# mengcaopku/DCNet

Measured on AMD Instinct MI355X. Metric: clips/sec (T=8, 416x416, bs8) fwd+bwd, higher is better.
Workload: dtype f32; 1 GPU; T=8 416x416 bs8/GPU L=20 fp32, 64 img/GPU/step as pairs, fwd+5 losses+bwd+RMSprop; arith=f16x2-split MFMA, fp32 accumulate, parallelism=dp1, ranks_seen=1, reducer=none, step=hipGraph replay (fwd+losses+bwd+RMSprop), sampler=mt

## Files before the change

### dcnet_amd/csrc/coattn.hip

```cpp
#include "igemm.h"
#include "prof.h"
#include "coattn.h"

int tn_gemm_batched(const float* A, int lda, long long a_bs, const float* B, int ldb, long long b_bs,
                    float* C, int ldc, long long c_bs, const float* row_scale,
                    int M, int m_ld, int N, int K, int batch, int accumulate, hipStream_t stream,
                    const unsigned* amax_a = nullptr, const unsigned* amax_b = nullptr);

namespace {

constexpr int EXP_ROWS = 32;

typedef _Float16 f16x4c_t __attribute__((ext_vector_type(4)));
constexpr float E_SPLIT_SCALE = 8192.f;
template <bool SPLIT>
__global__ __launch_bounds__(256) void exp_sums_kernel(float* __restrict__ E, int hw, int ldE, float t,
                                                       float* __restrict__ rsum, float* __restrict__ colpart) {
  __shared__ float red[4][EXP_ROWS];
  const int b = blockIdx.y, rb = blockIdx.x;
  const int i0 = rb * EXP_ROWS;
  float* e = E + ((size_t)b * hw + i0) * ldE;
  float racc[EXP_ROWS];
#pragma unroll
  for (int r = 0; r < EXP_ROWS; ++r) racc[r] = 0.f;
  const int nrow = min(EXP_ROWS, hw - i0);
  for (int j = threadIdx.x * 4; j < ldE; j += 1024) {
    f32x4 v[EXP_ROWS];
#pragma unroll
    for (int r = 0; r < EXP_ROWS; ++r)
      v[r] = r < nrow ? *reinterpret_cast<const f32x4*>(e + (size_t)r * ldE + j) : f32x4{0.f, 0.f, 0.f, 0.f};
    f32x4 cs = {0.f, 0.f, 0.f, 0.f};
#pragma unroll
    for (int r = 0; r < EXP_ROWS; ++r) {
      if (r < nrow) {
        f32x4 o;
#pragma unroll
        for (int k = 0; k < 4; ++k) o[k] = (j + k < hw) ? expf(t * v[r][k] - t) : 0.f;
        if constexpr (SPLIT) {
          const f32x4 ts = o * E_SPLIT_SCALE;
          const f16x4c_t h = {(_Float16)ts[0], (_Float16)ts[1], (_Float16)ts[2], (_Float16)ts[3]};
          const f16x4c_t l = {(_Float16)(ts[0] - (float)h[0]), (_Float16)(ts[1] - (float)h[1]), (_Float16)(ts[2] - (float)h[2]),
                              (_Float16)(ts[3] - (float)h[3])};
          unsigned char* run = reinterpret_cast<unsigned char*>(e + (size_t)r * ldE + (j & ~7)) + (j & 4) * 2;
          *reinterpret_cast<f16x4c_t*>(run) = h;
          *reinterpret_cast<f16x4c_t*>(run + 16) = l;
        } else {
          *reinterpret_cast<f32x4*>(e + (size_t)r * ldE + j) = o;
        }
        cs += o; racc[r] += (o[0] + o[1]) + (o[2] + o[3]);
      }
    }
    *reinterpret_cast<f32x4*>(colpart + ((size_t)rb * gridDim.y + b) * ldE + j) = cs;
  }
  const int lane = threadIdx.x & 63, wave = threadIdx.x >> 6;
#pragma unroll
  for (int r = 0; r < EXP_ROWS; ++r) {
    const float s = wave_sum(racc[r]);
    if (lane == 0) red[wave][r] = s;
  }
  __syncthreads();
  if (threadIdx.x < EXP_ROWS && i0 + threadIdx.x < hw)
    rsum[(size_t)b * hw + i0 + threadIdx.x] = 1.f / (red[0][threadIdx.x] + red[1][threadIdx.x] + red[2][threadIdx.x] + red[3][threadIdx.x]);
}

__global__ __launch_bounds__(256) void colsum_inv_kernel(const float* __restrict__ colpart, int nrb, int b, int hw, int ldE,
                                                         float* __restrict__ cinv) {
  const int j = blockIdx.x * 256 + threadIdx.x, bb = blockIdx.y;
  if (j >= hw) return;
  float s = 0.f;
  for (int rb = 0; rb < nrb; ++rb) s += colpart[((size_t)rb * b + bb) * ldE + j];
  cinv[(size_t)bb * hw + j] = 1.f / s;
}

enum { AM_ONE = 0, AM_DO1, AM_DO2, AM_DO1S, AM_DO2S, AM_DA, AM_DP1, AM_DP2, AM_SLOTS };
__global__ __launch_bounds__(256) void amax_init_kernel(unsigned* __restrict__ w) {
  for (int i = threadIdx.x; i < AM_SLOTS * DCN_AMAX_WORDS; i += 256) w[i] = i < DCN_AMAX_WORDS ? 0x3F800000u : 0u;
}

__global__ __launch_bounds__(256) void rowdot_scale_kernel(const float* __restrict__ d, int ldd, int64_t bsd,
                                                           const float* __restrict__ o, int ldo, int64_t bso, int hw,
                                                           const float* __restrict__ inv, int64_t rows, int c,
                                                           float* __restrict__ delta, float* __restrict__ ds,
                                                           unsigned* __restrict__ amax_d, unsigned* __restrict__ amax_ds) {
  __shared__ float red[4];
  const int lane = threadIdx.x & 63;
  const int64_t row = (int64_t)blockIdx.x * 4 + (threadIdx.x >> 6);
  float vmax = 0.f, s = 0.f;
  if (row < rows) {
    const int64_t bb = row / hw, i = row - bb * hw;
    s = inv[row];
    float acc = 0.f;
    for (int k = lane * 4; k < c; k += 256) {
      const f32x4 dv = *reinterpret_cast<const f32x4*>(d + bb * bsd + i * ldd + k);
      const f32x4 ov = *reinterpret_cast<const f32x4*>(o + bb * bso + i * ldo + k);
      acc += dv[0] * ov[0] + dv[1] * ov[1] + dv[2] * ov[2] + dv[3] * ov[3];
      *reinterpret_cast<f32x4*>(ds + row * c + k) = dv * s;
      vmax = fmaxf(fmaxf(vmax, fmaxf(fabsf(dv[0]), fabsf(dv[1]))), fmaxf(fabsf(dv[2]), fabsf(dv[3])));
    }
    acc = wave_sum(acc);
    if (lane == 0) delta[row] = acc;
  }
  const float vs = wave_max(vmax * s);
  amax_update_block(amax_d, vmax, red);
  __syncthreads();
  amax_update_block(amax_ds, vs, red);
}

template <bool ESPLIT, bool OSPLIT = false>
__global__ __launch_bounds__(256) void dA_kernel(const float* __restrict__ E, float* __restrict__ dP1, const float* __restrict__ dP2,
                                                 const float* __restrict__ rinv, const float* __restrict__ cinv,
                                                 const float* __restrict__ d1, const float* __restrict__ d2,
                                                 int hw, int ldE, float t, int64_t total4, unsigned* __restrict__ amax_da) {
  __shared__ float red[4];
  float vmax = 0.f;
  const int l4 = ldE >> 2;
  float s_out = 1.f;
  if constexpr (OSPLIT) {
    const int be = (int)((amax_read(amax_da) >> 23) & 0xFF);
    int ex = (be == 0 || be == 255) ? 0 : 14 - (be - 126);
    ex = ex > 100 ? 100 : (ex < -100 ? -100 : ex);
    s_out = __uint_as_float((unsigned)(ex + 127) << 23);
  }
  for (int64_t idx = (int64_t)blockIdx.x * 256 + threadIdx.x; idx < total4; idx += (int64_t)gridDim.x * 256) {
    const int64_t row = idx / l4;
    const int j = (int)(idx - row * l4) * 4;
    const int64_t bb = row / hw;
    f32x4 e;
    if constexpr (ESPLIT) {
      const unsigned char* run = reinterpret_cast<const unsigned char*>(E + row * ldE + (j & ~7)) + (j & 4) * 2;
      const f16x4c_t h = *reinterpret_cast<const f16x4c_t*>(run), l = *reinterpret_cast<const f16x4c_t*>(run + 16);
#pragma unroll
      for (int k = 0; k < 4; ++k) e[k] = ((float)h[k] + (float)l[k]) * (1.f / E_SPLIT_SCALE);
    } else {
      e = *reinterpret_cast<const f32x4*>(E + row * ldE + j);
    }
    const f32x4 p1 = *reinterpret_cast<const f32x4*>(dP1 + row * ldE + j);
    const f32x4 p2 = *reinterpret_cast<const f32x4*>(dP2 + row * ldE + j);
    const float ri = rinv[row], di = d1[row];
    f32x4 o;
#pragma unroll
    for (int k = 0; k < 4; ++k) {
      float v = 0.f;
      if (j + k < hw) v = t * e[k] * ((p1[k] - di) * ri + (p2[k] - d2[bb * hw + j + k]) * cinv[bb * hw + j + k]);
      o[k] = v;
    }
    if constexpr (OSPLIT) {
      const f32x4 ts = o * s_out;
      const f16x4c_t h = {(_Float16)ts[0], (_Float16)ts[1], (_Float16)ts[2], (_Float16)ts[3]};
      const f16x4c_t l = {(_Float16)(ts[0] - (float)h[0]), (_Float16)(ts[1] - (float)h[1]), (_Float16)(ts[2] - (float)h[2]),
                          (_Float16)(ts[3] - (float)h[3])};
      unsigned char* run = reinterpret_cast<unsigned char*>(dP1 + row * ldE + (j & ~7)) + (j & 4) * 2;
      *reinterpret_cast<f16x4c_t*>(run) = h;
      *reinterpret_cast<f16x4c_t*>(run + 16) = l;
    } else {
      *reinterpret_cast<f32x4*>(dP1 + row * ldE + j) = o;
      vmax = fmaxf(fmaxf(vmax, fmaxf(fabsf(o[0]), fabsf(o[1]))), fmaxf(fabsf(o[2]), fabsf(o[3])));
    }
  }
  if constexpr (!OSPLIT) amax_update_block(amax_da, vmax, red);
}

__global__ __launch_bounds__(64) void da_bound_kernel(const unsigned* __restrict__ a1, const unsigned* __restrict__ a2, float t,
                                                      unsigned* __restrict__ out) {
  const float b = 2.f * t * (__uint_as_float(amax_read(a1)) + __uint_as_float(amax_read(a2)));
  out[threadIdx.x & (DCN_AMAX_WORDS - 1)] = __float_as_uint(b);
}

inline int ld_pad(int hw) { return (hw + 31) / 32 * 32; }

void gemm_params(IgemmParams& p, const float* A, int lda, long long a_bs, const float* B, int ldb, long long b_bs,
                 float* C, int ldc, long long c_bs, int M, int N, int K, int batch) {
  p = IgemmParams{};
  p.osy = p.osx = p.isy = p.isx = 1; p.dense_out = 1;
  p.in = A; p.ldi = lda; p.in_bs = a_bs; p.wt = B; p.ldw = ldb; p.wt_bs = b_bs; p.out = C; p.ldo = ldc; p.out_bs = c_bs;
  p.ldr = ldc;
  p.N = 1; p.Hi = 1; p.Wi = M; p.Ho = 1; p.Wo = M; p.Hs = 1; p.Ws = M; p.M = M;
  p.Ci = K; p.Co = N; p.ntaps = 1; p.batch = batch;
}

}

static bool on_gemm3(int b, int hw, int c) { return c % 32 == 0 && gemm3_applicable(hw, c, hw, b) && gemm3_applicable(hw, hw, c, b); }

int coattn_ld_pad(int hw) { return ld_pad(hw); }
bool coattn_on_gemm3(int b, int hw, int c) { return on_gemm3(b, hw, c); }
unsigned* coattn_ws_amax(float* ws, int b, int hw) { return reinterpret_cast<unsigned*>(ws + (int64_t)cdiv(hw, EXP_ROWS) * b * ld_pad(hw)); }
int coattn_amax_init(unsigned* am, hipStream_t stream) {
  hipLaunchKernelGGL(amax_init_kernel, dim3(1), dim3(256), 0, stream, am);
  DCN_CHECK_LAUNCH("coattn amax_init");
  return DCN_OK;
}
int coattn_exp_sums(float* E, int b, int hw, float temperature, float* rinv, float* cinv, float* ws, bool split, hipStream_t stream) {
  const int ldE = ld_pad(hw), nrb = cdiv(hw, EXP_ROWS);
  const int pid = prof_begin(12, (double)b * hw * ldE * 8.0, stream);
  if (split) hipLaunchKernelGGL(exp_sums_kernel<true>, dim3(nrb, b), dim3(256), 0, stream, E, hw, ldE, temperature, rinv, ws);
  else hipLaunchKernelGGL(exp_sums_kernel<false>, dim3(nrb, b), dim3(256), 0, stream, E, hw, ldE, temperature, rinv, ws);
  prof_end(pid, stream);
  DCN_CHECK_LAUNCH("exp_sums");
  hipLaunchKernelGGL(colsum_inv_kernel, dim3(cdiv(hw, 256), b), dim3(256), 0, stream, ws, nrb, b, hw, ldE, cinv);
  DCN_CHECK_LAUNCH("colsum_inv");
  return DCN_OK;
}

extern "C" int64_t dcn_coattn_fwd_ws(int b, int hw, int c) {
  (void)c;
  return (int64_t)cdiv(hw, EXP_ROWS) * b * ld_pad(hw) + AM_SLOTS * DCN_AMAX_WORDS;
}
extern "C" int64_t dcn_coattn_e_size(int b, int hw) { return (int64_t)b * hw * ld_pad(hw); }
extern "C" int64_t dcn_coattn_saved_size(int b, int hw, int c) {
  return dcn_coattn_e_size(b, hw) + (on_gemm3(b, hw, c) ? (int64_t)2 * b * hw * c : 0);
}

extern "C" int dcn_coattn_fwd(const float* f1, const float* f2, int ldf, int64_t bsf, float* f1_attn, float* f2_attn, int ldo,
                              int64_t bso, float* E, float* rinv, float* cinv, float* ws,
                              int b, int hw, int c, float temperature, void* stream_) {
  hipStream_t stream = (hipStream_t)stream_;
  DCN_CHECK_ARG(f1 && f2 && f1_attn && E && rinv && cinv && ws, "coattn_fwd: null pointer");
  DCN_CHECK_ARG(b > 0 && hw > 0 && c > 0 && c % 32 == 0, "coattn_fwd: bad shape (c=%d must be a multiple of 32)", c);
  if (ldf <= 0) ldf = c;
  if (ldo <= 0) ldo = c;
  DCN_CHECK_ARG(ldf % 4 == 0 && ldo % 4 == 0, "coattn_fwd: ldf/ldo must be multiples of 4");
  if (bsf <= 0) bsf = (int64_t)hw * ldf;
  if (bso <= 0) bso = (int64_t)hw * ldo;
  DCN_CHECK_ARG(bsf % 4 == 0 && bso % 4 == 0, "coattn_fwd: batch strides must be multiples of 4");
  const int ldE = ld_pad(hw);
  unsigned* am = reinterpret_cast<unsigned*>(ws + (int64_t)cdiv(hw, EXP_ROWS) * b * ldE);
  hipLaunchKernelGGL(amax_init_kernel, dim3(1), dim3(256), 0, stream, am);
  DCN_CHECK_LAUNCH("coattn amax_init");
  const unsigned* one = am + AM_ONE * DCN_AMAX_WORDS;
  const int nrb = cdiv(hw, EXP_ROWS);
  const long long bsE = (long long)hw * ldE;
  if (on_gemm3(b, hw, c)) {
    float* f1s = E + dcn_coattn_e_size(b, hw);
    float* f2s = f1s + (int64_t)b * hw * c;
    const long long bss = (long long)hw * c;
    int rc = gemm3_presplit(f1, ldf, bsf, f1s, c, bss, b, hw, c, one, stream);
    if (rc) return rc;
    if ((rc = gemm3_presplit(f2, ldf, bsf, f2s, c, bss, b, hw, c, one, stream))) return rc;
    if ((rc = gemm3_launch(f1s, c, bss, 0, f2s, c, bss, 0, E, ldE, bsE, nullptr, 0, hw, hw, c, b, 0, one, one, stream))) return rc;
    const int pid = prof_begin(12, (double)b * hw * ldE * 8.0, stream);
    hipLaunchKernelGGL(exp_sums_kernel<true>, dim3(nrb, b), dim3(256), 0, stream, E, hw, ldE, temperature, rinv, ws);
    prof_end(pid, stream);
    DCN_CHECK_LAUNCH("exp_sums");
    hipLaunchKernelGGL(colsum_inv_kernel, dim3(cdiv(hw, 256), b), dim3(256), 0, stream, ws, nrb, b, hw, ldE, cinv);
    DCN_CHECK_LAUNCH("colsum_inv");
    if ((rc = gemm3_launch(E, ldE, bsE, 0, f2s, c, bss, 1, f1_attn, ldo, bso, rinv, hw, hw, c, hw, b, 0, one, one, stream))) return rc;
    if (f2_attn) rc = gemm3_launch(E, ldE, bsE, 1, f1s, c, bss, 1, f2_attn, ldo, bso, cinv, hw, hw, c, hw, b, 0, one, one, stream);
    return rc;
  }
  IgemmParams p;
  gemm_params(p, f1, ldf, bsf, f2, ldf, bsf, E, ldE, (long long)hw * ldE, hw, hw, c, b);
  p.amax_a = one; p.amax_b = one;
  int rc = igemm_launch(p, stream);
  if (rc) return rc;
  const int pid = prof_begin(12, (double)b * hw * ldE * 8.0, stream);
  hipLaunchKernelGGL(exp_sums_kernel<false>, dim3(nrb, b), dim3(256), 0, stream, E, hw, ldE, temperature, rinv, ws);
  prof_end(pid, stream);
  DCN_CHECK_LAUNCH("exp_sums");
  hipLaunchKernelGGL(colsum_inv_kernel, dim3(cdiv(hw, 256), b), dim3(256), 0, stream, ws, nrb, b, hw, ldE, cinv);
  DCN_CHECK_LAUNCH("colsum_inv");
  gemm_params(p, E, ldE, (long long)hw * ldE, f2, ldf, bsf, f1_attn, ldo, bso, hw, c, ldE, b);
  p.bmode = 1; p.kvalid = hw; p.row_scale = rinv; p.amax_a = one; p.amax_b = one;
  rc = igemm_launch(p, stream);
  if (rc) return rc;
  if (f2_attn)
    rc = tn_gemm_batched(E, ldE, (long long)hw * ldE, f1, ldf, bsf, f2_attn, ldo, bso,
                         cinv, hw, ldE, c, hw, b, 0, stream, one, one);
  return rc;
}

extern "C" int64_t dcn_coattn_bwd_ws(int b, int hw, int c) {
  return (int64_t)2 * b * hw * ld_pad(hw) + (int64_t)2 * b * hw * c + (int64_t)2 * b * hw + AM_SLOTS * DCN_AMAX_WORDS +
         (on_gemm3(b, hw, c) ? (int64_t)2 * b * hw * c + 4 : 0);
}

extern "C" int dcn_coattn_bwd(const float* f1, const float* f2, int ldf, int64_t bsf,
                              const float* d_f1_attn, const float* d_f2_attn, int lddo, int64_t bsdo,
                              const float* f1_attn, const float* f2_attn, int ldo, int64_t bso,
                              const float* E, const float* rinv, const float* cinv,
                              float* d_f1, float* d_f2, int lddf, int64_t bsdf, int accumulate, float* ws,
                              int b, int hw, int c, float temperature, void* stream_) {
  hipStream_t stream = (hipStream_t)stream_;
  DCN_CHECK_ARG(f1 && f2 && d_f1_attn && d_f2_attn && f1_attn && f2_attn && E && rinv && cinv && d_f1 && d_f2 && ws,
                "coattn_bwd: null pointer");
  DCN_CHECK_ARG(b > 0 && hw > 0 && c > 0 && c % 32 == 0, "coattn_bwd: bad shape");
  if (ldf <= 0) ldf = c;
  if (ldo <= 0) ldo = c;
  if (lddo <= 0) lddo = c;
  if (lddf <= 0) lddf = c;
  if (bsf <= 0) bsf = (int64_t)hw * ldf;
  if (bso <= 0) bso = (int64_t)hw * ldo;
  if (bsdo <= 0) bsdo = (int64_t)hw * lddo;
  if (bsdf <= 0) bsdf = (int64_t)hw * lddf;
  const int ldE = ld_pad(hw);
  const long long rows = (long long)b * hw;
  float* dP1 = ws;
  float* dP2 = dP1 + rows * ldE;
  float* dO1s = dP2 + rows * ldE;
  float* dO2s = dO1s + rows * c;
  float* del1 = dO2s + rows * c;
  float* del2 = del1 + rows;
  unsigned* am = reinterpret_cast<unsigned*>(del2 + rows);
  hipLaunchKernelGGL(amax_init_kernel, dim3(1), dim3(256), 0, stream, am);
  DCN_CHECK_LAUNCH("coattn amax_init");
  auto slot = [&](int i) { return am + i * DCN_AMAX_WORDS; };
  hipLaunchKernelGGL(rowdot_scale_kernel, dim3(cdiv(rows, 4)), dim3(256), 0, stream, d_f1_attn, lddo, bsdo, f1_attn, ldo, bso, hw, rinv, rows, c, del1, dO1s,
                     slot(AM_DO1), slot(AM_DO1S));
  DCN_CHECK_LAUNCH("rowdot_scale");
  hipLaunchKernelGGL(rowdot_scale_kernel, dim3(cdiv(rows, 4)), dim3(256), 0, stream, d_f2_attn, lddo, bsdo, f2_attn, ldo, bso, hw, cinv, rows, c, del2, dO2s,
                     slot(AM_DO2), slot(AM_DO2S));
  DCN_CHECK_LAUNCH("rowdot_scale");
  const int64_t total4 = rows * (ldE / 4);
  int64_t g = (total4 + 255) / 256; if (g > 8192) g = 8192;
  if (g > 1024) g = 1024;
  const long long bsE = (long long)hw * ldE;
  if (on_gemm3(b, hw, c)) {
    float* dO1p = reinterpret_cast<float*>(((uintptr_t)(am + AM_SLOTS * DCN_AMAX_WORDS) + 15) & ~(uintptr_t)15);
    float* dO2p = dO1p + rows * c;
    const float* f1s = E + dcn_coattn_e_size(b, hw);
    const float* f2s = f1s + rows * c;
    const long long bss = (long long)hw * c;
    int rc;
    if ((rc = gemm3_presplit(d_f1_attn, lddo, bsdo, dO1p, c, bss, b, hw, c, slot(AM_DO1), stream))) return rc;
    if ((rc = gemm3_presplit(d_f2_attn, lddo, bsdo, dO2p, c, bss, b, hw, c, slot(AM_DO2), stream))) return rc;
    if ((rc = gemm3_presplit(dO1s, c, bss, dO1s, c, bss, b, hw, c, slot(AM_DO1S), stream))) return rc;
    if ((rc = gemm3_presplit(dO2s, c, bss, dO2s, c, bss, b, hw, c, slot(AM_DO2S), stream))) return rc;
    if ((rc = gemm3_launch(dO1p, c, bss, 0, f2s, c, bss, 0, dP1, ldE, bsE, nullptr, 0, hw, hw, c, b, 0, slot(AM_DO1), slot(AM_ONE), stream, slot(AM_DP1)))) return rc;
    if ((rc = gemm3_launch(f1s, c, bss, 0, dO2p, c, bss, 0, dP2, ldE, bsE, nullptr, 0, hw, hw, c, b, 0, slot(AM_ONE), slot(AM_DO2), stream, slot(AM_DP2)))) return rc;
    hipLaunchKernelGGL(da_bound_kernel, dim3(1), dim3(64), 0, stream, slot(AM_DP1), slot(AM_DP2), temperature, slot(AM_DA));
    DCN_CHECK_LAUNCH("dA bound");
    const int pid_da = prof_begin(31, (double)total4 * 16.0 * 4.0, stream);
    hipLaunchKernelGGL((dA_kernel<true, true>), dim3((int)g), dim3(256), 0, stream, E, dP1, dP2, rinv, cinv, del1, del2, hw, ldE, temperature, total4, slot(AM_DA));
    prof_end(pid_da, stream);
    DCN_CHECK_LAUNCH("dA");
    if ((rc = gemm3_launch(dP1, ldE, bsE, 0, f2s, c, bss, 1, d_f1, lddf, bsdf, nullptr, 0, hw, c, hw, b, accumulate, slot(AM_DA), slot(AM_ONE), stream))) return rc;
    if ((rc = gemm3_launch(E, ldE, bsE, 0, dO2s, c, bss, 1, d_f1, lddf, bsdf, nullptr, 0, hw, c, hw, b, 1, slot(AM_ONE), slot(AM_DO2S), stream))) return rc;
    if ((rc = gemm3_launch(dP1, ldE, bsE, 1, f1s, c, bss, 1, d_f2, lddf, bsdf, nullptr, 0, hw, c, hw, b, accumulate, slot(AM_DA), slot(AM_ONE), stream))) return rc;
    return gemm3_launch(E, ldE, bsE, 1, dO1s, c, bss, 1, d_f2, lddf, bsdf, nullptr, 0, hw, c, hw, b, 1, slot(AM_ONE), slot(AM_DO1S), stream);
  }
  IgemmParams p;
  int rc;
  gemm_params(p, d_f1_attn, lddo, bsdo, f2, ldf, bsf, dP1, ldE, (long long)hw * ldE, hw, hw, c, b);
  p.amax_a = slot(AM_DO1); p.amax_b = slot(AM_ONE);
  if ((rc = igemm_launch(p, stream))) return rc;
  gemm_params(p, f1, ldf, bsf, d_f2_attn, lddo, bsdo, dP2, ldE, (long long)hw * ldE, hw, hw, c, b);
  p.amax_a = slot(AM_ONE); p.amax_b = slot(AM_DO2);
  if ((rc = igemm_launch(p, stream))) return rc;
  const int pid_da = prof_begin(31, (double)total4 * 16.0 * 4.0, stream);
  hipLaunchKernelGGL(dA_kernel<false>, dim3((int)g), dim3(256), 0, stream, E, dP1, dP2, rinv, cinv, del1, del2, hw, ldE, temperature, total4, slot(AM_DA));
  prof_end(pid_da, stream);
  DCN_CHECK_LAUNCH("dA");
  gemm_params(p, dP1, ldE, (long long)hw * ldE, f2, ldf, bsf, d_f1, lddf, bsdf, hw, c, ldE, b);
  p.bmode = 1; p.kvalid = hw; p.accumulate = accumulate; p.amax_a = slot(AM_DA); p.amax_b = slot(AM_ONE);
  if ((rc = igemm_launch(p, stream))) return rc;
  gemm_params(p, E, ldE, (long long)hw * ldE, dO2s, c, (long long)hw * c, d_f1, lddf, bsdf, hw, c, ldE, b);
  p.bmode = 1; p.kvalid = hw; p.accumulate = 1; p.amax_a = slot(AM_ONE); p.amax_b = slot(AM_DO2S);
  if ((rc = igemm_launch(p, stream))) return rc;
  rc = tn_gemm_batched(dP1, ldE, (long long)hw * ldE, f1, ldf, bsf, d_f2, lddf, bsdf,
                       nullptr, hw, ldE, c, hw, b, accumulate, stream, slot(AM_DA), slot(AM_ONE));
  if (rc) return rc;
  return tn_gemm_batched(E, ldE, (long long)hw * ldE, dO1s, c, (long long)hw * c, d_f2, lddf, bsdf,
                         nullptr, hw, ldE, c, hw, b, 1, stream, slot(AM_ONE), slot(AM_DO1S));
}
```

### dcnet_amd/csrc/gemm3.hip

```cpp
#include "igemm.h"
#include "prof.h"

namespace {

typedef _Float16 f16x8_t __attribute__((ext_vector_type(8)));
typedef short s16x4 __attribute__((ext_vector_type(4)));
typedef short s16x8 __attribute__((ext_vector_type(8)));
typedef __attribute__((address_space(3))) void lds_void;

#ifndef G3_ABL
#define G3_ABL 0
#endif
constexpr unsigned G3_OOB = 0x80000000u;
constexpr int G3_BM = 256, G3_BN = 256, G3_STAGES = 4;
constexpr int G3_TILE = 256 * 64;
constexpr int G3_STAGE = 2 * G3_TILE;
constexpr int G3_LDS = G3_STAGES * G3_STAGE;

__device__ __forceinline__ float g3_pow2_scale(unsigned amax_bits) {
  const int be = (int)((amax_bits >> 23) & 0xFF);
  if (be == 0 || be == 255) return 1.f;
  int e = 14 - (be - 126);
  e = e > 100 ? 100 : (e < -100 ? -100 : e);
  return __uint_as_float((unsigned)(e + 127) << 23);
}

struct G3Params {
  const float* A; const float* B; float* C;
  long long a_bs, b_bs, c_bs;
  int lda, ldb, ldc;
  int M, N, K;
  int a_rows, b_rows;
  int a_cols, b_cols;
  int tiles_m, tiles_n;
  const float* row_scale; long long rs_bs;
  int accumulate;
  const unsigned* amax_a; const unsigned* amax_b;
  unsigned* amax_out;
  int var;
  int abl;
};

__device__ __forceinline__ int g3_tswz(int krow) { return (krow & 1) | ((krow & 2) << 1); }

template <bool AT, bool BT, bool H1 = false>
__global__ __launch_bounds__(512, 1) void gemm3_kernel(const G3Params p) {
  extern __shared__ __attribute__((aligned(1024))) unsigned char smem3g[];
  const int tid = threadIdx.x, lane = tid & 63;
  const int wave = __builtin_amdgcn_readfirstlane(tid >> 6);
  const int wm = wave >> 2, wn = wave & 3;
  const int per_batch = p.tiles_m * p.tiles_n;
  const int lin = xcd_remap(blockIdx.x, gridDim.x);
  const int batch = __builtin_amdgcn_readfirstlane(lin / per_batch), t_ = lin - batch * per_batch;
  const int bm = __builtin_amdgcn_readfirstlane(t_ / p.tiles_n), bn = t_ - bm * p.tiles_n;
  const int m0 = bm * G3_BM, n0 = bn * G3_BN;
  const int kslices = (p.K + 15) >> 4;

  const float* a_base = p.A + batch * p.a_bs + (AT ? 0 : (long long)m0 * p.lda);
  const float* b_base = p.B + batch * p.b_bs + (BT ? 0 : (long long)n0 * p.ldb);
  const int a_rows_left = AT ? p.a_rows : p.a_rows - m0, b_rows_left = BT ? p.b_rows : p.b_rows - n0;
  const long long a_bytes = ((long long)(a_rows_left - 1) * p.lda + p.a_cols) * 4, b_bytes = ((long long)(b_rows_left - 1) * p.ldb + p.b_cols) * 4;
  const __amdgpu_buffer_rsrc_t a_rs = __builtin_amdgcn_make_buffer_rsrc((void*)a_base, 0, a_bytes > 0x7FFFFFF0LL ? 0x7FFFFFF0 : (int)a_bytes, 0x00020000);
  const __amdgpu_buffer_rsrc_t b_rs = __builtin_amdgcn_make_buffer_rsrc((void*)b_base, 0, b_bytes > 0x7FFFFFF0LL ? 0x7FFFFFF0 : (int)b_bytes, 0x00020000);

  unsigned voff[4];
  int sstep_a, sstep_b;
#pragma unroll
  for (int e = 0; e < 2; ++e) {
    const int j = 2 * wave + e;
    if (AT) {
      voff[e] = (unsigned)((long long)j * p.lda * 4 + m0 * 4 + ((lane ^ g3_tswz(j)) << 4));
      if (m0 + ((lane ^ g3_tswz(j)) << 2) >= p.a_cols) voff[e] = G3_OOB;
    } else {
      const int row = 16 * j + (lane >> 2), c = (lane & 3) ^ ((row >> 2) & 3);
      voff[e] = row < a_rows_left ? (unsigned)((long long)row * p.lda * 4 + c * 16) : G3_OOB;
    }
    if (BT) {
      voff[2 + e] = (unsigned)((long long)j * p.ldb * 4 + n0 * 4 + ((lane ^ g3_tswz(j)) << 4));
      if (n0 + ((lane ^ g3_tswz(j)) << 2) >= p.b_cols) voff[2 + e] = G3_OOB;
    } else {
      const int row = 16 * j + (lane >> 2), c = (lane & 3) ^ ((row >> 2) & 3);
      voff[2 + e] = row < b_rows_left ? (unsigned)((long long)row * p.ldb * 4 + c * 16) : G3_OOB;
    }
  }
  sstep_a = AT ? 16 * p.lda * 4 : 64;
  sstep_b = BT ? 16 * p.ldb * 4 : 64;
  const int my_dst = 2 * wave * 1024;

  int k_done = 0;
  auto issue_a = [&]() {
    const bool live = k_done < kslices && !(G3_ABL && (p.abl & 1));
    unsigned char* st = smem3g + (k_done & (G3_STAGES - 1)) * G3_STAGE + my_dst;
    int sa_ = live ? k_done * sstep_a : 0;
    if (G3_ABL && (p.abl & 8)) sa_ = 0;
#pragma unroll
    for (int e = 0; e < 2; ++e)
      __builtin_amdgcn_raw_ptr_buffer_load_lds(a_rs, (lds_void*)(st + e * 1024), 16, (int)(live ? voff[e] : G3_OOB), sa_, 0, 0);
  };
  auto issue_b = [&]() {
    const bool live = k_done < kslices && !(G3_ABL && (p.abl & 1));
    unsigned char* st = smem3g + (k_done & (G3_STAGES - 1)) * G3_STAGE + my_dst;
    int sb_ = live ? k_done * sstep_b : 0;
    if (G3_ABL && (p.abl & 8)) sb_ = 0;
#pragma unroll
    for (int e = 0; e < 2; ++e)
      __builtin_amdgcn_raw_ptr_buffer_load_lds(b_rs, (lds_void*)(st + G3_TILE + e * 1024), 16, (int)(live ? voff[2 + e] : G3_OOB), sb_, 0, 0);
    ++k_done;
  };
  auto issue = [&]() { issue_a(); issue_b(); };

  const int g = lane >> 5;
  const int hh = lane >> 5, gg = (lane >> 4) & 1, qq = (lane & 15) >> 2, pp = lane & 3;
  int a_rd[4][2], b_rd[2][2];
#pragma unroll
  for (int mi = 0; mi < 4; ++mi) {
    if (AT) {
      const int c = wm * 128 + mi * 32 + 16 * gg + 4 * pp;
#pragma unroll
      for (int r2 = 0; r2 < 2; ++r2) {
        const int kr = 8 * hh + 4 * r2 + qq;
        a_rd[mi][r2] = kr * 1024 + ((((c >> 3) * 2) ^ g3_tswz(kr)) << 4) + (c & 7) * 2;
      }
    } else {
      const int ar = wm * 128 + mi * 32 + (lane & 31);
      a_rd[mi][0] = ar * 64 + (((2 * g) ^ ((ar >> 2) & 3)) << 4);
      a_rd[mi][1] = ar * 64 + (((2 * g + 1) ^ ((ar >> 2) & 3)) << 4);
    }
  }
#pragma unroll
  for (int ni = 0; ni < 2; ++ni) {
    if (BT) {
      const int c = wn * 64 + ni * 32 + 16 * gg + 4 * pp;
#pragma unroll
      for (int r2 = 0; r2 < 2; ++r2) {
        const int kr = 8 * hh + 4 * r2 + qq;
        b_rd[ni][r2] = G3_TILE + kr * 1024 + ((((c >> 3) * 2) ^ g3_tswz(kr)) << 4) + (c & 7) * 2;
      }
    } else {
      const int br = wn * 64 + ni * 32 + (lane & 31);
      b_rd[ni][0] = G3_TILE + br * 64 + (((2 * g) ^ ((br >> 2) & 3)) << 4);
      b_rd[ni][1] = G3_TILE + br * 64 + (((2 * g + 1) ^ ((br >> 2) & 3)) << 4);
    }
  }
  auto tr_read = [&](const unsigned char* ptr) {
    return __builtin_amdgcn_ds_read_tr16_b64_v4i16((__attribute__((address_space(3))) s16x4*)(ptr));
  };
  auto tfrag = [&](const unsigned char* st, int off0, int off1, int plane) {
    const s16x4 lo = tr_read(st + (off0 ^ (plane << 4))), hi = tr_read(st + (off1 ^ (plane << 4)));
    const s16x8 v = {lo[0], lo[1], lo[2], lo[3], hi[0], hi[1], hi[2], hi[3]};
    return __builtin_bit_cast(f16x8_t, v);
  };

  f32x16 acc[4][2];
#pragma unroll
  for (int mi = 0; mi < 4; ++mi)
#pragma unroll
    for (int ni = 0; ni < 2; ++ni)
#pragma unroll
      for (int r = 0; r < 16; ++r) acc[mi][ni][r] = 0.f;

  for (int s = 0; s < G3_STAGES - 1; ++s) issue();

  asm volatile("s_waitcnt vmcnt(%0)" :: "n"((G3_STAGES - 2) * 4) : "memory");
  if (wm == 1) __builtin_amdgcn_s_barrier();
  for (int it = 0; it < kslices; ++it) {
    __builtin_amdgcn_s_barrier();
    asm volatile("" ::: "memory");
    const unsigned char* st = smem3g + (it & (G3_STAGES - 1)) * G3_STAGE;
    f16x8_t bh[2], bl[2];
    f16x8_t ah[4], al[4];
    if (G3_ABL && (p.abl & 2)) {
#pragma unroll
      for (int ni = 0; ni < 2; ++ni) { bh[ni] = f16x8_t{(_Float16)it, 0, 0, 0, 0, 0, 0, 0}; bl[ni] = bh[ni]; }
#pragma unroll
      for (int mi = 0; mi < 4; ++mi) { ah[mi] = bh[0]; al[mi] = bh[1]; }
    } else {
#pragma unroll
      for (int ni = 0; ni < 2; ++ni) {
        if (BT) { bh[ni] = tfrag(st, b_rd[ni][0], b_rd[ni][1], 0); if constexpr (!H1) bl[ni] = tfrag(st, b_rd[ni][0], b_rd[ni][1], 1); }
        else { bh[ni] = *reinterpret_cast<const f16x8_t*>(st + b_rd[ni][0]); if constexpr (!H1) bl[ni] = *reinterpret_cast<const f16x8_t*>(st + b_rd[ni][1]); }
      }
#pragma unroll
      for (int mi = 0; mi < 4; ++mi) {
        if (AT) { ah[mi] = tfrag(st, a_rd[mi][0], a_rd[mi][1], 0); if constexpr (!H1) al[mi] = tfrag(st, a_rd[mi][0], a_rd[mi][1], 1); }
        else { ah[mi] = *reinterpret_cast<const f16x8_t*>(st + a_rd[mi][0]); if constexpr (!H1) al[mi] = *reinterpret_cast<const f16x8_t*>(st + a_rd[mi][1]); }
      }
    }
    if (p.var >= 1) {
      issue_a();
      if (wm == 1) asm volatile("s_waitcnt vmcnt(%0)" :: "n"((G3_STAGES - 2) * 4 - 2) : "memory");
    } else {
      issue();
      if (wm == 1) asm volatile("s_waitcnt vmcnt(%0)" :: "n"((G3_STAGES - 2) * 4) : "memory");
    }
    asm volatile("s_waitcnt lgkmcnt(0)" ::: "memory");
    __builtin_amdgcn_s_barrier();
    asm volatile("" ::: "memory");
    if (G3_ABL && (p.abl & 4)) {
#pragma unroll
      for (int mi = 0; mi < 4; ++mi) { asm volatile("" :: "v"(ah[mi]), "v"(al[mi])); }
#pragma unroll
      for (int ni = 0; ni < 2; ++ni) { asm volatile("" :: "v"(bh[ni]), "v"(bl[ni])); }
    } else {
      __builtin_amdgcn_s_setprio(1);
      if constexpr (!H1) {
#pragma unroll
        for (int mi = 0; mi < 4; ++mi)
#pragma unroll
          for (int ni = 0; ni < 2; ++ni) acc[mi][ni] = __builtin_amdgcn_mfma_f32_32x32x16_f16(al[mi], bh[ni], acc[mi][ni], 0, 0, 0);
        if (p.var == 2) issue_b();
#pragma unroll
        for (int mi = 0; mi < 4; ++mi)
#pragma unroll
          for (int ni = 0; ni < 2; ++ni) acc[mi][ni] = __builtin_amdgcn_mfma_f32_32x32x16_f16(ah[mi], bl[ni], acc[mi][ni], 0, 0, 0);
      } else if (p.var == 2) issue_b();
#pragma unroll
      for (int mi = 0; mi < 4; ++mi)
#pragma unroll
        for (int ni = 0; ni < 2; ++ni) acc[mi][ni] = __builtin_amdgcn_mfma_f32_32x32x16_f16(ah[mi], bh[ni], acc[mi][ni], 0, 0, 0);
      __builtin_amdgcn_s_setprio(0);
    }
    if (p.var == 1) issue_b();
    if (wm == 0) asm volatile("s_waitcnt vmcnt(%0)" :: "n"((G3_STAGES - 2) * 4) : "memory");
  }
  if (wm == 0) __builtin_amdgcn_s_barrier();
  asm volatile("s_waitcnt vmcnt(0)" ::: "memory");

  const float dq = 1.f / (g3_pow2_scale(amax_read(p.amax_a)) * g3_pow2_scale(amax_read(p.amax_b)));
  float* __restrict__ cb = p.C + batch * p.c_bs;
  const float* rs = p.row_scale ? p.row_scale + batch * p.rs_bs : nullptr;
  float vmax = 0.f;
#pragma unroll
  for (int mi = 0; mi < 4; ++mi)
#pragma unroll
    for (int r = 0; r < 16; ++r) {
      const int m = m0 + wm * 128 + mi * 32 + 4 * g + (r & 3) + 8 * (r >> 2);
      if (m >= p.M) continue;
      const float f = rs ? dq * rs[m] : dq;
#pragma unroll
      for (int ni = 0; ni < 2; ++ni) {
        const int n = n0 + wn * 64 + ni * 32 + (lane & 31);
        if (n >= p.N) continue;
        float v = acc[mi][ni][r] * f;
        float* dst = cb + (long long)m * p.ldc + n;
        if (p.accumulate) v += *dst;
        *dst = v;
        vmax = fmaxf(vmax, fabsf(v));
      }
    }
  if (p.amax_out) {
    vmax = wave_max(vmax);
    if (lane == 0) amax_update(p.amax_out, vmax, blockIdx.x * 8 + wave);
  }
}

__global__ __launch_bounds__(256) void presplit_kernel(const float* __restrict__ src, int ld, long long bs, float* __restrict__ dst, int ldd,
                                                        long long bsd, int rows, int c, long long total8, const unsigned* __restrict__ amax) {
  const float s = g3_pow2_scale(amax_read(amax));
  const int c8 = c >> 3;
  for (long long i = (long long)blockIdx.x * 256 + threadIdx.x; i < total8; i += (long long)gridDim.x * 256) {
    const long long row_all = i / c8; const int o = (int)(i - row_all * c8);
    const long long b = row_all / rows; const int row = (int)(row_all - b * rows);
    const float* sp = src + b * bs + (long long)row * ld + o * 8;
    const f32x4 x0 = *reinterpret_cast<const f32x4*>(sp) * s, x1 = *reinterpret_cast<const f32x4*>(sp + 4) * s;
    f16x8_t h, l;
#pragma unroll
    for (int e = 0; e < 4; ++e) { h[e] = (_Float16)x0[e]; h[4 + e] = (_Float16)x1[e]; }
#pragma unroll
    for (int e = 0; e < 4; ++e) { l[e] = (_Float16)(x0[e] - (float)h[e]); l[4 + e] = (_Float16)(x1[e] - (float)h[4 + e]); }
    float* dp = dst + b * bsd + (long long)row * ldd + o * 8;
    *reinterpret_cast<f16x8_t*>(dp) = h;
    *reinterpret_cast<f16x8_t*>(dp + 4) = l;
  }
}

DCN_KNOB(g_gemm3, "Gemm3", 1, "gemm3.hip: the co-attention products on pre-split operands (0 = implicit-GEMM / weight-gradient tiles; + 256 * v = schedule variant v; + 16 * bits = timing ablations, results WRONG)",
         nullptr, "-DG3_ABL=1", G3_ABL != 0, [](int v) { return (v & 0xF0) != 0; });
DCN_KNOB(g_gemm3_h1, "H1gemm3", 1, "gemm3.hip: one f16 piece per operand in the bf16 precision modes (0 = both pieces, fp32-accurate co-attention)");

template <bool AT, bool BT, bool H1>
int launch3g_(const G3Params& p, int grid, hipStream_t stream) {
  static DcnPerDeviceFlag attr_once;
  if (attr_once.first()) {
    (void)hipFuncSetAttribute(reinterpret_cast<const void*>(&gemm3_kernel<AT, BT, H1>), hipFuncAttributeMaxDynamicSharedMemorySize, G3_LDS);
  }
  hipLaunchKernelGGL((gemm3_kernel<AT, BT, H1>), dim3(grid), dim3(512), G3_LDS, stream, p);
  return DCN_OK;
}
template <bool AT, bool BT>
int launch3g(const G3Params& p, int grid, hipStream_t stream) {
  if (g_gemm3_h1 && igemm_precision() == 2) return launch3g_<AT, BT, true>(p, grid, stream);
  return launch3g_<AT, BT, false>(p, grid, stream);
}

}

int gemm3_variant() { const int v = g_gemm3 >> 8; return (v == 1 || v == 2) ? v : 0; }
extern "C" int dcn_gemm3_variant() { return gemm3_variant(); }

bool gemm3_applicable(int M, int N, int K, int batch) {
  return g_gemm3 && (igemm_precision() == 4 || igemm_precision() == 2) && M >= 512 && N >= 256 && K >= 64 && batch >= 1;
}

int gemm3_presplit(const float* src, int ld, long long bs, float* dst, int ldd, long long bsd, int batch, int rows, int c,
                   const unsigned* amax, hipStream_t stream) {
  DCN_CHECK_ARG(src && dst && amax && c % 8 == 0 && ld % 4 == 0 && ldd % 4 == 0 && bs % 4 == 0 && bsd % 4 == 0, "gemm3_presplit: bad argument");
  const long long total8 = (long long)batch * rows * (c / 8);
  long long g = (total8 + 255) / 256; if (g > 16384) g = 16384;
  hipLaunchKernelGGL(presplit_kernel, dim3((int)g), dim3(256), 0, stream, src, ld, bs, dst, ldd, bsd, rows, c, total8, amax);
  DCN_CHECK_LAUNCH("gemm3_presplit");
  return DCN_OK;
}

int gemm3_launch(const float* A, int lda, long long a_bs, int at, const float* B, int ldb, long long b_bs, int bt,
                 float* C, int ldc, long long c_bs, const float* row_scale, long long rs_bs,
                 int M, int N, int K, int batch, int accumulate, const unsigned* amax_a, const unsigned* amax_b, hipStream_t stream,
                 unsigned* amax_out) {
  DCN_CHECK_ARG(A && B && C && amax_a && amax_b, "gemm3: null pointer");
  DCN_CHECK_ARG(lda % 4 == 0 && ldb % 4 == 0 && a_bs % 4 == 0 && b_bs % 4 == 0 && (((uintptr_t)A | (uintptr_t)B) & 15) == 0, "gemm3: 16-byte rows");
  G3Params p{};
  p.A = A; p.B = B; p.C = C; p.a_bs = a_bs; p.b_bs = b_bs; p.c_bs = c_bs; p.lda = lda; p.ldb = ldb; p.ldc = ldc;
  p.M = M; p.N = N; p.K = K;
  const int k16 = (K + 15) / 16 * 16;
  p.a_rows = at ? K : M; p.b_rows = bt ? K : N;
  p.a_cols = at ? (M + 7) / 8 * 8 : k16; p.b_cols = bt ? (N + 7) / 8 * 8 : k16;
  DCN_CHECK_ARG(p.a_cols <= lda && p.b_cols <= ldb, "gemm3: rows shorter than the tile reads (lda=%d ldb=%d)", lda, ldb);
  p.tiles_m = cdiv(M, G3_BM); p.tiles_n = cdiv(N, G3_BN);
  p.row_scale = row_scale; p.rs_bs = rs_bs; p.accumulate = accumulate; p.amax_a = amax_a; p.amax_b = amax_b; p.amax_out = amax_out; p.abl = (g_gemm3 >> 4) & 15; p.var = gemm3_variant();
  const int grid = p.tiles_m * p.tiles_n * batch;
  const int pid = prof_begin(40, 2.0 * batch * (double)M * N * K, stream);
  int rc;
  if (at) rc = bt ? launch3g<true, true>(p, grid, stream) : DCN_ERR_ARG;
  else rc = bt ? launch3g<false, true>(p, grid, stream) : launch3g<false, false>(p, grid, stream);
  prof_end(pid, stream);
  DCN_CHECK_ARG(rc == DCN_OK, "gemm3: no A^T . B^T form");
  DCN_CHECK_LAUNCH("gemm3");
  return DCN_OK;
}

extern "C" int dcn_gemm3_supported(int m, int n, int k, int batch) { return gemm3_applicable(m, n, k, batch) ? 1 : 0; }

extern "C" int dcn_gemm3_presplit(const float* src, int ld, int64_t bs, float* dst, int ldd, int64_t bsd, int batch, int rows, int c,
                                  const uint32_t* amax, void* stream) {
  return gemm3_presplit(src, ld, bs, dst, ldd, bsd, batch, rows, c, amax, (hipStream_t)stream);
}

extern "C" int dcn_gemm3(const float* a, int lda, int64_t a_bs, int a_t, const float* b, int ldb, int64_t b_bs, int b_t,
                         float* c, int ldc, int64_t c_bs, const float* row_scale, int64_t rs_bs,
                         int m, int n, int k, int batch, int accumulate, const uint32_t* amax_a, const uint32_t* amax_b, void* stream) {
  DCN_CHECK_ARG(m > 0 && n > 0 && k > 0 && batch > 0, "gemm3: empty problem");
  return gemm3_launch(a, lda, a_bs, a_t, b, ldb, b_bs, b_t, c, ldc, c_bs, row_scale, rs_bs, m, n, k, batch, accumulate, amax_a, amax_b,
                      (hipStream_t)stream, nullptr);
}
```

### dcnet_amd/csrc/igemm.h

```cpp
#pragma once
#include "common.h"

#define IGEMM_MAX_TAPS 16


struct IgemmParams {
  const float* in;
  const float* wt;
  const float* f8;
  const unsigned* amax_a;
  const unsigned* amax_b;
  const void* wt16;
  const float* b_scale;
  unsigned* amax_out;
  float* out;
  const float* scale;
  const float* shift;
  const float* residual;
  float* stats;
  const float* row_scale;
  int batch;
  long long in_bs, wt_bs, out_bs;
  int bmode;
  int kvalid;
  int N, Hi, Wi, Ci, ldi;
  int Ho, Wo;
  int Hs, Ws;
  int oy0, ox0, osy, osx;
  int isy, isx;
  int Co, ldo, ldr, ldw;
  int M;
  int ntaps;
  int cpt, kiters;
  int act; float slope;
  int accumulate, dense_out, c4;
  int tap_dy[IGEMM_MAX_TAPS], tap_dx[IGEMM_MAX_TAPS], tap_w[IGEMM_MAX_TAPS];
  int ncls;
  int cls_M[4], cls_Hs[4], cls_Ws[4], cls_oy0[4], cls_ox0[4], cls_ntaps[4];
  const float* bt_y; const float* bt_mean; const float* bt_invstd; const float* bt_gamma; const float* bt_beta;
  int bt_act; float bt_slope;
  const unsigned char* a_scale8; const unsigned char* b_scale8;
};
inline double epilogue_reads(const IgemmParams& p) { return 1.0 + (p.accumulate ? 1.0 : 0.0) + (p.residual ? 1.0 : 0.0) + (p.bt_y ? 1.0 : 0.0); }
bool igemm_tap_capable(const IgemmParams& p);

int igemm_grid_m(int M, int Co, int ntaps);
int igemm_launch(const IgemmParams& p, hipStream_t stream);
bool igemm_will_presplit(long long rows, int Co, int ntaps, int Ci);

bool conv3_applicable(const IgemmParams& p, int precision, int gran);
int conv3_launch(const IgemmParams& p, int gran, hipStream_t stream);
bool conv3x_takes(const IgemmParams& p, int gran);
int conv3x_launch(const IgemmParams& p, int gran, hipStream_t stream);
int conv3b_bm(int M, int Co, int Wi);
bool conv3b_takes(const IgemmParams& p);
int conv3b_launch(const IgemmParams& p, int out_f32, hipStream_t stream);

bool conv1_applicable(const IgemmParams& p, int precision, int gran);
int conv1_launch(const IgemmParams& p, int gran, hipStream_t stream);
int conv1_tile_of(long long rows, int Co, int ntaps, int Ci, int stats, int gran, int storage16);
int conv1b_grid_m(int M, int Co, int ntaps, int s1_w = 0);
int conv1b_launch(const IgemmParams& p, int out_f32, hipStream_t stream);
int conv1q_grid_m(int M, int Co);
int conv1q_launch(const IgemmParams& p, int out_f32, hipStream_t stream);
bool conv2b_takes(int M, int Co, int ntaps);
int conv2b_launch(const IgemmParams& p, int out_f32, hipStream_t stream);


bool stem_applicable(const IgemmParams& p, const float* scratch);
int stem_launch(const IgemmParams& p, float* scratch, hipStream_t stream);

bool dgrad2_applicable(int n, int h, int wd, int cin, int cout, int ksize, int stride, int accumulate);
struct DcnBnTap { const float* y; const float* mean; const float* invstd; const float* gamma; const float* beta; int act; float slope;
                  float* stats; int stats_rows; };
int nconv1_launch_b16(int mode, const void* x, int ldi, const void* w16, void* y, int ldo, float* stats, int stats_rows,
                      int n, int h, int wd, int stride, hipStream_t stream);
int dgrad2_launch_b16(const void* dy, int lddy, const void* wt16, void* dx, int n, int h, int wd, int cin, int accumulate, hipStream_t stream);
int dgrad2_grid(int n, int h, int wd, int cin);
int dgrad2_launch(const float* dy, int lddy, const float* wt, float* dx, int n, int h, int wd, int cin, int accumulate,
                  const uint32_t* amax_dy, const uint32_t* amax_w, const DcnBnTap* tap, hipStream_t stream);
bool gemm3_applicable(int M, int N, int K, int batch);
int gemm3_presplit(const float* src, int ld, long long bs, float* dst, int ldd, long long bsd, int batch, int rows, int c,
                   const unsigned* amax, hipStream_t stream);
int gemm3_launch(const float* A, int lda, long long a_bs, int at, const float* B, int ldb, long long b_bs, int bt,
                 float* C, int ldc, long long c_bs, const float* row_scale, long long rs_bs,
                 int M, int N, int K, int batch, int accumulate, const unsigned* amax_a, const unsigned* amax_b, hipStream_t stream,
                 unsigned* amax_out = nullptr);
int igemm_precision();
extern int g_abl;
extern int g_wsplit;
struct DcnPreAct { const float* scale; const float* shift; int act; float slope; };
bool nconv1_applicable(int mode, int n, int h, int wd, int cin, int cout, int ksize, int stride);
int nconv1_launch(int mode, const float* x, int ldi, const float* w, float* y, int ldo, float* stats, int stats_rows,
                  int n, int h, int wd, int stride, const uint32_t* amax_x, const uint32_t* amax_w, const DcnPreAct* pre, hipStream_t stream);
```

Measured before the change: 88.57 clips/s.

## Fuse exp, f16 split and row/column partial sums into the affinity GEMM epilogue

The co-attention affinity GEMM (gemm3 NT path) now applies exp(t*s - t) in its epilogue. It writes E directly in the f16 hi/lo split layout and emits per-32-row column partial sums plus per-quad row partials. This removes the separate exp_sums pass, which re-read and re-wrote the full E matrix. A small rowsum_inv kernel then reduces the quad partials into row inverses. The change adds an extra workspace buffer and more epilogue register pressure and DPP shuffling in the GEMM.

New measurement: 88.75 clips/s (median of 6 runs). Within noise of the previous version (+0.2%).

```diff
diff --git a/dcnet_amd/csrc/coattn.hip b/dcnet_amd/csrc/coattn.hip
--- a/dcnet_amd/csrc/coattn.hip
+++ b/dcnet_amd/csrc/coattn.hip
@@ -70,6 +70,21 @@
   float s = 0.f;
   for (int rb = 0; rb < nrb; ++rb) s += colpart[((size_t)rb * b + bb) * ldE + j];
   cinv[(size_t)bb * hw + j] = 1.f / s;
+}
+
+__global__ __launch_bounds__(256) void rowsum_inv_kernel(const float* __restrict__ quad, int ldE, int64_t rows, float* __restrict__ rinv) {
+  const int lane = threadIdx.x & 63, ldq = ldE >> 2;
+  const int64_t row = (int64_t)blockIdx.x * 4 + (threadIdx.x >> 6);
+  if (row >= rows) return;
+  const float* q = quad + row * ldq;
+  float s[4];
+#pragma unroll
+  for (int w = 0; w < 4; ++w) {
+    float racc = 0.f;
+    for (int j = 64 * w + lane; j < ldq; j += 256) racc += q[j];
+    s[w] = wave_sum(racc);
+  }
+  if (lane == 0) rinv[row] = 1.f / (s[0] + s[1] + s[2] + s[3]);
 }
 
 enum { AM_ONE = 0, AM_DO1, AM_DO2, AM_DO1S, AM_DO2S, AM_DA, AM_DP1, AM_DP2, AM_SLOTS };
@@ -202,9 +217,9 @@
   return DCN_OK;
 }
 
+static int64_t fwd_ws_quads(int b, int hw) { return (int64_t)cdiv(hw, EXP_ROWS) * b * ld_pad(hw) + AM_SLOTS * DCN_AMAX_WORDS; }
 extern "C" int64_t dcn_coattn_fwd_ws(int b, int hw, int c) {
-  (void)c;
-  return (int64_t)cdiv(hw, EXP_ROWS) * b * ld_pad(hw) + AM_SLOTS * DCN_AMAX_WORDS;
+  return fwd_ws_quads(b, hw) + (on_gemm3(b, hw, c) ? (int64_t)b * hw * (ld_pad(hw) / 4) : 0);
 }
 extern "C" int64_t dcn_coattn_e_size(int b, int hw) { return (int64_t)b * hw * ld_pad(hw); }
 extern "C" int64_t dcn_coattn_saved_size(int b, int hw, int c) {
@@ -237,11 +252,11 @@
     int rc = gemm3_presplit(f1, ldf, bsf, f1s, c, bss, b, hw, c, one, stream);
     if (rc) return rc;
     if ((rc = gemm3_presplit(f2, ldf, bsf, f2s, c, bss, b, hw, c, one, stream))) return rc;
-    if ((rc = gemm3_launch(f1s, c, bss, 0, f2s, c, bss, 0, E, ldE, bsE, nullptr, 0, hw, hw, c, b, 0, one, one, stream))) return rc;
-    const int pid = prof_begin(12, (double)b * hw * ldE * 8.0, stream);
-    hipLaunchKernelGGL(exp_sums_kernel<true>, dim3(nrb, b), dim3(256), 0, stream, E, hw, ldE, temperature, rinv, ws);
-    prof_end(pid, stream);
-    DCN_CHECK_LAUNCH("exp_sums");
+    Gemm3Epi ep{};
+    ep.t = temperature; ep.colpart = ws; ep.quad = ws + fwd_ws_quads(b, hw);
+    if ((rc = gemm3_launch(f1s, c, bss, 0, f2s, c, bss, 0, E, ldE, bsE, nullptr, 0, hw, hw, c, b, 0, one, one, stream, nullptr, &ep))) return rc;
+    hipLaunchKernelGGL(rowsum_inv_kernel, dim3(cdiv((long long)b * hw, 4)), dim3(256), 0, stream, ep.quad, ldE, (int64_t)b * hw, rinv);
+    DCN_CHECK_LAUNCH("rowsum_inv");
     hipLaunchKernelGGL(colsum_inv_kernel, dim3(cdiv(hw, 256), b), dim3(256), 0, stream, ws, nrb, b, hw, ldE, cinv);
     DCN_CHECK_LAUNCH("colsum_inv");
     if ((rc = gemm3_launch(E, ldE, bsE, 0, f2s, c, bss, 1, f1_attn, ldo, bso, rinv, hw, hw, c, hw, b, 0, one, one, stream))) return rc;
diff --git a/dcnet_amd/csrc/gemm3.hip b/dcnet_amd/csrc/gemm3.hip
--- a/dcnet_amd/csrc/gemm3.hip
+++ b/dcnet_amd/csrc/gemm3.hip
@@ -12,7 +12,7 @@
 #define G3_ABL 0
 #endif
 constexpr unsigned G3_OOB = 0x80000000u;
-constexpr int G3_BM = 256, G3_BN = 256, G3_STAGES = 4;
+constexpr int G3_BM = GEMM3_TILE, G3_BN = GEMM3_TILE, G3_STAGES = 4;
 constexpr int G3_TILE = 256 * 64;
 constexpr int G3_STAGE = 2 * G3_TILE;
 constexpr int G3_LDS = G3_STAGES * G3_STAGE;
@@ -39,11 +39,22 @@
   unsigned* amax_out;
   int var;
   int abl;
+  Gemm3Epi epi;
 };
 
+__device__ __forceinline__ unsigned g3_pair_swap(unsigned mine, unsigned sel) {
+  const unsigned other = (unsigned)__builtin_amdgcn_mov_dpp((int)mine, 0xB1, 0xF, 0xF, true);
+  return __builtin_amdgcn_perm(other, mine, sel);
+}
+__device__ __forceinline__ unsigned g3_split_bits(float ts) {
+  const _Float16 h = (_Float16)ts, l = (_Float16)(ts - (float)h);
+  return (unsigned)__builtin_bit_cast(unsigned short, h) | ((unsigned)__builtin_bit_cast(unsigned short, l) << 16);
+}
+constexpr float G3_E_SCALE = 8192.f;
+
 __device__ __forceinline__ int g3_tswz(int krow) { return (krow & 1) | ((krow & 2) << 1); }
 
-template <bool AT, bool BT, bool H1 = false>
+template <bool AT, bool BT, bool H1 = false, int EPI = 0>
 __global__ __launch_bounds__(512, 1) void gemm3_kernel(const G3Params p) {
   extern __shared__ __attribute__((aligned(1024))) unsigned char smem3g[];
   const int tid = threadIdx.x, lane = tid & 63;
@@ -228,6 +239,50 @@
 
   const float dq = 1.f / (g3_pow2_scale(amax_read(p.amax_a)) * g3_pow2_scale(amax_read(p.amax_b)));
   float* __restrict__ cb = p.C + batch * p.c_bs;
+  if constexpr (EPI != 0) {
+    const int odd = lane & 1;
+    const unsigned sel = odd ? 0x03020706u : 0x05040100u;
+    const float t = p.epi.t;
+    const int ldq = p.ldc >> 2, nbatch = gridDim.x / per_batch;
+#pragma unroll
+    for (int mi = 0; mi < 4; ++mi) {
+      const int mb = m0 + wm * 128 + mi * 32;
+      float o[16][2];
+#pragma unroll
+      for (int r = 0; r < 16; ++r) {
+        const int m = mb + 4 * g + (r & 3) + 8 * (r >> 2);
+        const bool mrow = m < p.M;
+#pragma unroll
+        for (int ni = 0; ni < 2; ++ni) {
+          const int n = n0 + wn * 64 + ni * 32 + (lane & 31);
+          o[r][ni] = (mrow && n < p.N) ? expf(t * (acc[mi][ni][r] * dq) - t) : 0.f;
+          const unsigned w = g3_pair_swap(g3_split_bits(o[r][ni] * G3_E_SCALE), sel);
+          float q2 = o[r][ni] + __builtin_bit_cast(float, __builtin_amdgcn_mov_dpp(__builtin_bit_cast(int, o[r][ni]), 0xB1, 0xF, 0xF, true));
+          q2 += __builtin_bit_cast(float, __builtin_amdgcn_mov_dpp(__builtin_bit_cast(int, q2), 0x4E, 0xF, 0xF, true));
+          if (mrow && n < p.ldc) {
+            *reinterpret_cast<unsigned*>(reinterpret_cast<unsigned char*>(cb + (long long)m * p.ldc + (n & ~7)) + odd * 16 + ((n & 7) >> 1) * 4) = w;
+            if ((lane & 3) == 0) p.epi.quad[((long long)batch * p.M + m) * ldq + (n >> 2)] = q2;
+          }
+        }
+      }
+      if (mb < p.M) {
+#pragma unroll
+        for (int ni = 0; ni < 2; ++ni) {
+          const int n = n0 + wn * 64 + ni * 32 + (lane & 31);
+          float cs = 0.f;
+#pragma unroll
+          for (int q = 0; q < 8; ++q) {
+            const int r = 4 * (q >> 1);
+            const float mine = (((cs + o[r][ni]) + o[r + 1][ni]) + o[r + 2][ni]) + o[r + 3][ni];
+            const float other = __shfl_xor(mine, 32);
+            cs = g == (q & 1) ? mine : other;
+          }
+          if (g == 0 && n < p.ldc) p.epi.colpart[((long long)(mb >> 5) * nbatch + batch) * p.ldc + n] = cs;
+        }
+      }
+    }
+    return;
+  }
   const float* rs = p.row_scale ? p.row_scale + batch * p.rs_bs : nullptr;
   float vmax = 0.f;
 #pragma unroll
@@ -278,19 +333,19 @@
          nullptr, "-DG3_ABL=1", G3_ABL != 0, [](int v) { return (v & 0xF0) != 0; });
 DCN_KNOB(g_gemm3_h1, "H1gemm3", 1, "gemm3.hip: one f16 piece per operand in the bf16 precision modes (0 = both pieces, fp32-accurate co-attention)");
 
-template <bool AT, bool BT, bool H1>
+template <bool AT, bool BT, bool H1, int EPI>
 int launch3g_(const G3Params& p, int grid, hipStream_t stream) {
   static DcnPerDeviceFlag attr_once;
   if (attr_once.first()) {
-    (void)hipFuncSetAttribute(reinterpret_cast<const void*>(&gemm3_kernel<AT, BT, H1>), hipFuncAttributeMaxDynamicSharedMemorySize, G3_LDS);
-  }
-  hipLaunchKernelGGL((gemm3_kernel<AT, BT, H1>), dim3(grid), dim3(512), G3_LDS, stream, p);
+    (void)hipFuncSetAttribute(reinterpret_cast<const void*>(&gemm3_kernel<AT, BT, H1, EPI>), hipFuncAttributeMaxDynamicSharedMemorySize, G3_LDS);
+  }
+  hipLaunchKernelGGL((gemm3_kernel<AT, BT, H1, EPI>), dim3(grid), dim3(512), G3_LDS, stream, p);
   return DCN_OK;
 }
-template <bool AT, bool BT>
+template <bool AT, bool BT, int EPI = 0>
 int launch3g(const G3Params& p, int grid, hipStream_t stream) {
-  if (g_gemm3_h1 && igemm_precision() == 2) return launch3g_<AT, BT, true>(p, grid, stream);
-  return launch3g_<AT, BT, false>(p, grid, stream);
+  if (g_gemm3_h1 && igemm_precision() == 2) return launch3g_<AT, BT, true, EPI>(p, grid, stream);
+  return launch3g_<AT, BT, false, EPI>(p, grid, stream);
 }
 
 }
@@ -315,9 +370,12 @@
 int gemm3_launch(const float* A, int lda, long long a_bs, int at, const float* B, int ldb, long long b_bs, int bt,
                  float* C, int ldc, long long c_bs, const float* row_scale, long long rs_bs,
                  int M, int N, int K, int batch, int accumulate, const unsigned* amax_a, const unsigned* amax_b, hipStream_t stream,
-                 unsigned* amax_out) {
+                 unsigned* amax_out, const Gemm3Epi* epi) {
   DCN_CHECK_ARG(A && B && C && amax_a && amax_b, "gemm3: null pointer");
-  DCN_CHECK_ARG(lda % 4 == 0 && ldb % 4 == 0 && a_bs % 4 == 0 && b_bs % 4 == 0 && (((uintptr_t)A | (uintptr_t)B) & 15) == 0, "gemm3: 16-byte rows");
+  if (epi) {
+    DCN_CHECK_ARG(!at && !bt && !row_scale && !amax_out && !accumulate && epi->colpart && epi->quad, "gemm3: the affinity epilogue belongs to the plain NT product");
+    DCN_CHECK_ARG(ldc % 32 == 0 && c_bs % 8 == 0 && ((uintptr_t)C & 31) == 0 && N <= ldc && M == N, "gemm3: the affinity epilogue writes square E with rows padded to 32 (ldc=%d)", ldc);
+  }
   G3Params p{};
   p.A = A; p.B = B; p.C = C; p.a_bs = a_bs; p.b_bs = b_bs; p.c_bs = c_bs; p.lda = lda; p.ldb = ldb; p.ldc = ldc;
   p.M = M; p.N = N; p.K = K;
@@ -328,9 +386,11 @@
   p.tiles_m = cdiv(M, G3_BM); p.tiles_n = cdiv(N, G3_BN);
   p.row_scale = row_scale; p.rs_bs = rs_bs; p.accumulate = accumulate; p.amax_a = amax_a; p.amax_b = amax_b; p.amax_out = amax_out; p.abl = (g_gemm3 >> 4) & 15; p.var = gemm3_variant();
   const int grid = p.tiles_m * p.tiles_n * batch;
+  if (epi) p.epi = *epi;
   const int pid = prof_begin(40, 2.0 * batch * (double)M * N * K, stream);
   int rc;
-  if (at) rc = bt ? launch3g<true, true>(p, grid, stream) : DCN_ERR_ARG;
+  if (epi) rc = launch3g<false, false, 1>(p, grid, stream);
+  else if (at) rc = bt ? launch3g<true, true>(p, grid, stream) : DCN_ERR_ARG;
   else rc = bt ? launch3g<false, true>(p, grid, stream) : launch3g<false, false>(p, grid, stream);
   prof_end(pid, stream);
   DCN_CHECK_ARG(rc == DCN_OK, "gemm3: no A^T . B^T form");
diff --git a/dcnet_amd/csrc/igemm.h b/dcnet_amd/csrc/igemm.h
--- a/dcnet_amd/csrc/igemm.h
+++ b/dcnet_amd/csrc/igemm.h
@@ -80,12 +80,14 @@
 int dgrad2_launch(const float* dy, int lddy, const float* wt, float* dx, int n, int h, int wd, int cin, int accumulate,
                   const uint32_t* amax_dy, const uint32_t* amax_w, const DcnBnTap* tap, hipStream_t stream);
 bool gemm3_applicable(int M, int N, int K, int batch);
+constexpr int GEMM3_TILE = 256;
 int gemm3_presplit(const float* src, int ld, long long bs, float* dst, int ldd, long long bsd, int batch, int rows, int c,
                    const unsigned* amax, hipStream_t stream);
+struct Gemm3Epi { float t; float* colpart; float* quad; };
 int gemm3_launch(const float* A, int lda, long long a_bs, int at, const float* B, int ldb, long long b_bs, int bt,
                  float* C, int ldc, long long c_bs, const float* row_scale, long long rs_bs,
                  int M, int N, int K, int batch, int accumulate, const unsigned* amax_a, const unsigned* amax_b, hipStream_t stream,
-                 unsigned* amax_out = nullptr);
+                 unsigned* amax_out = nullptr, const Gemm3Epi* epi = nullptr);
 int igemm_precision();
 extern int g_abl;
 extern int g_wsplit;
```
